# araffin/robotics-rl-srl

Measured on NVIDIA H100. Metric: env-steps/sec KukaButtonGymEnv-v0 ground_truth @4096 envs/GPU, higher is better.
Workload: dtype f32

## Files before the change

### robotics-rl-srl_b200/csrc/kuka_coop.cuh

```cuda
#pragma once
#include <math.h>
#include <stdint.h>
#include "kuka_params.cuh"

#if defined(__CUDACC__)
#define KC_F __device__ __forceinline__
#else
#define KC_F inline
#endif
#if defined(__CUDA_ARCH__)
#define KC_RSQRT(x) rsqrtf(x)
#else
#define KC_RSQRT(x) (1.0f / sqrtf(x))
#endif

#define KC_G 4
#define KC_BS 53
#define KC_CS 25

enum {
    KB_R = 0,
    KB_N = 0,
    KB_F = 3,
    KB_PM = 6,
// ... 344 lines not shown
    for (int t = 0; t < 4; ++t) {
        const int idx = 4 * u + t;
        const int f = idx < 10 ? KB_M + idx : KB_N + (idx - 10);
        float v[KK_NB];
#pragma unroll
        for (int j = 0; j < KK_NB; ++j) v[j] = s[j * KC_BS + f];
#pragma unroll
        for (int j = KK_NB - 1; j >= 1; --j) v[j == 10 ? 7 : j - 1] += v[j];
#pragma unroll
        for (int j = 0; j < KK_NB - 1; ++j)
            if (j != 9) s[j * KC_BS + f] = v[j];
    }
}
template <class S>
KC_F void kc_ph_mass(const S& s, int u) {
    kc3 a[KK_NB], pv[KK_NB];
#pragma unroll
    for (int i = 0; i < KK_NB; ++i) { a[i] = kc_ld3(s, i * KC_BS + KB_A); pv[i] = kc_ld3(s, i * KC_BS + KB_PV); }
#pragma unroll
    for (int k = 0; k < KK_NB / KC_G; ++k) {
        const int j = u + KC_G * k, o = j * KC_BS;
        const kc3 aj = kc_ld3(s, o + KB_A), pvj = kc_ld3(s, o + KB_PV);
        const kc3 h = kc_ld3(s, o + KB_H);
        s[KC_OFF_BIAS + j] = kc_dot(aj, kc_ld3(s, o + KB_N)) + kc_dot(pvj, kc_ld3(s, o + KB_F));
        float I[6];
#pragma unroll
        for (int t = 0; t < 6; ++t) I[t] = s[o + KB_IO + t];
        const kc3 Pm = kc_fma(s[o + KB_M], pvj, kc_cross(aj, h));
        const kc3 Lm = kc_add(kc_symv(I, aj), kc_cross(h, pvj));
#pragma unroll
        for (int i = 0; i < KK_NB; ++i) {
            if (i > 4 * k + 3) continue;
            const float val = kc_anc(i, j) ? kc_dot(a[i], Lm) + kc_dot(pv[i], Pm) : 0.f;
            if (i < 4 * k || i <= j) s[KC_OFF_MA + j * KC_MS + i] = val;
        }
    }
}

template <bool TWOB, bool SCALED, class S>
KC_F void kc_ph_rows(const S& s, const KukaParams& P, const float (&A)[KK_NB][KK_NB], int nc, int u, const float* tgt = nullptr) {
#pragma unroll 1
    for (int r = u; r < 3 * nc; r += KC_G) {
        const int c = r < nc ? r : (r - nc) >> 1;
        const int co = KC_OFF_CT + c * KC_CTS, ro = KC_OFF_ROWS + r * KC_RS;
        const kc3 n = kc_ld3(s, co + 3), pt = kc_ld3(s, co + 6);
        kc3 dir = n;
        if (r >= nc) {
            kc3 t1, t2;
            if (fabsf(n.z) > 0.70710678f) {
                const float a = n.y * n.y + n.z * n.z, kk = KC_RSQRT(a);
                t1 = kc_mk(0.f, -n.z * kk, n.y * kk); t2 = kc_mk(a * kk, -n.x * t1.z, n.x * t1.y);
            } else {
                const float a = n.x * n.x + n.y * n.y, kk = KC_RSQRT(a);
                t1 = kc_mk(-n.y * kk, n.x * kk, 0.f); t2 = kc_mk(-n.z * t1.y, n.z * t1.x, a * kk);
            }
            dir = ((r - nc) & 1) ? t2 : t1;
        }
        const int body = (int)s[co], shape = (int)s[co + 1];
        float J[KK_NB];
#pragma unroll
        for (int j = 0; j < KK_NB; ++j)
            J[j] = kc_anc(j, body) ? kc_dot(dir, kc_cross(kc_ld3(s, j * KC_BS + KB_A), kc_sub(pt, kc_ld3(s, j * KC_BS + KB_P)))) : 0.f;
        const float jb = shape == 1 ? -dir.z : 0.f, jb2 = TWOB && shape == 3 ? -dir.z : 0.f;
        float D = 0.f, off = 0.f;
#pragma unroll
        for (int i = 0; i < KK_NB; ++i) {
            float acc = 0.f;
#pragma unroll
            for (int j = 0; j < KK_NB; ++j) acc = fmaf(i >= j ? A[i][j] : A[j][i], J[j], acc);
            D = fmaf(J[i], acc, D);
            if (SCALED) off = fmaf(J[i], tgt[i], off);
            s[ro + KK_ROW_J + i] = SCALED ? J[i] * P.sat_isig[i] : J[i];
            s[ro + KK_ROW_W + i] = SCALED ? acc * P.sat_sig[i] : acc;
            if (SCALED && r < nc) s[KC_OFF_WT + 4 * i + r] = acc * P.sat_sig[i];
        }
        s[ro + KK_ROW_J + KK_NB] = jb; s[ro + KK_ROW_W + KK_NB] = jb * P.btn_minv;
        s[ro + KK_ROW_J + KK_NB + 1] = jb2; s[ro + KK_ROW_W + KK_NB + 1] = jb2 * P.btn_minv;
        D = fmaf(jb, jb * P.btn_minv, D);
        if (TWOB) D = fmaf(jb2, jb2 * P.btn_minv, D);
        s[ro + KK_ROW_INVD] = 1.0f / D;
        const float pen = s[co + 2];
        s[ro + KK_ROW_TGT] = (r < nc ? (pen > 0.f ? -pen * P.inv_dt : -P.erp * pen * P.inv_dt) : 0.f) - off;
    }
    if (SCALED && u >= nc) {
#pragma unroll
        for (int i = 0; i < KK_NB; ++i) s[KC_OFF_WT + 4 * i + u] = 0.f;
    }
}

#if defined(__CUDACC__)
#define KC_RUN(call) do { call; __syncwarp(gmask); } while (0)
#else
#define KC_RUN(call) do { for (int u = 0; u < KC_G; ++u) { call; } } while (0)
#endif

#if defined(__CUDACC__)
template <bool TWOB, class S>
KC_F bool kc_kinematics(const S& s, const float* tab, const KukaParams& P, const KcKinIn& in, int u, unsigned gmask) {
    KC_RUN(kc_ph_local(s, tab, in, u));
    KC_RUN(kc_ph_chain(s, tab, P, u));
    const bool near = kc_ph_body<TWOB>(s, tab, P, in, u);
    __syncwarp(gmask);
    if (near) KC_RUN((kc_ph_collect<TWOB>(s, tab, P, u)));
    return near;
}
#else
template <bool TWOB, class S>
KC_F bool kc_kinematics(const S& s, const float* tab, const KukaParams& P, const KcKinIn& in) {
    KC_RUN(kc_ph_local(s, tab, in, u));
    KC_RUN(kc_ph_chain(s, tab, P, u));
    bool near = false;
    for (int u = 0; u < KC_G; ++u) near = kc_ph_body<TWOB>(s, tab, P, in, u);
    if (near) KC_RUN((kc_ph_collect<TWOB>(s, tab, P, u)));
    return near;
}
#endif

#if defined(__CUDACC__)
template <class S>
KC_F void kc_dynamics(const S& s, const KukaParams& P, const float* qd, int u, unsigned gmask) {
#else
template <class S>
KC_F void kc_dynamics(const S& s, const KukaParams& P, const float* qd) {
#endif
    KC_RUN(kc_ph_vel_terms(s, qd, u));
    KC_RUN(kc_ph_prefix2(s, KB_W, KB_VO, 0.f, u));
    KC_RUN(kc_ph_acc_terms(s, qd, u));
    KC_RUN(kc_ph_prefix2(s, KB_AW, KB_AV, -P.gz, u));
    KC_RUN(kc_ph_wrench(s, P, u));
    KC_RUN(kc_ph_subtree(s, u));
    KC_RUN(kc_ph_mass(s, u));
}
```

### robotics-rl-srl_b200/csrc/kuka_device.cuh

```cuda
#pragma once
#include <math.h>
#include <stdint.h>
#include "kuka_params.cuh"
#include "philox.cuh"
#include "kuka_coop.cuh"

#define KK_DEV __device__ __forceinline__

#if defined(KK_TIMING)
#define KK_PROBE_D(d) kk_probe_any |= ((d) != 0.f);
#define KK_PROBE_SWEEP() { ++kk_probe_sweep; if (!kk_probe_any && !kk_probe_conv) kk_probe_conv = kk_probe_sweep; kk_probe_any = false; }
#else
#define KK_PROBE_D(d)
#define KK_PROBE_SWEEP()
#endif
enum { KK_PH_KIN = 0, KK_PH_IK, KK_PH_DYN, KK_PH_CHOL, KK_PH_SETUP, KK_PH_FAST, KK_PH_GENERAL, KK_PH_ENV, KK_NPH };
#if defined(KK_PHASES) && defined(__CUDACC__)
struct KkPhaseClock { long long last; long long acc[KK_NPH]; };
#define KK_PH(clk, k) do { if (clk) { const long long t_ = clock64(); (clk)->acc[k] += t_ - (clk)->last; (clk)->last = t_; } } while (0)
#else
struct KkPhaseClock { long long dummy; };
#define KK_PH(clk, k) do { (void)(clk); } while (0)
#endif
struct f3 { float x, y, z; };
struct alignas(16) kk_f4 { float x, y, z, w; };
KK_DEV f3 mk3(float x, float y, float z) { f3 r; r.x = x; r.y = y; r.z = z; return r; }
KK_DEV f3 operator+(f3 a, f3 b) { return mk3(a.x + b.x, a.y + b.y, a.z + b.z); }
KK_DEV f3 operator-(f3 a, f3 b) { return mk3(a.x - b.x, a.y - b.y, a.z - b.z); }
KK_DEV f3 operator*(float s, f3 a) { return mk3(s * a.x, s * a.y, s * a.z); }
KK_DEV float dot3(f3 a, f3 b) { return fmaf(a.x, b.x, fmaf(a.y, b.y, a.z * b.z)); }
KK_DEV f3 cross3(f3 a, f3 b) { return mk3(a.y * b.z - a.z * b.y, a.z * b.x - a.x * b.z, a.x * b.y - a.y * b.x); }
KK_DEV float norm3(f3 a) { return sqrtf(dot3(a, a)); }
KK_DEV f3 symv(const float* I, f3 v) {
    return mk3(I[0] * v.x + I[1] * v.y + I[2] * v.z, I[1] * v.x + I[3] * v.y + I[4] * v.z, I[2] * v.x + I[4] * v.y + I[5] * v.z);
}

#define KK_PAR(i) ((i) == 0 ? -1 : (i) == 10 ? 7 : (i) - 1)

struct KukaEnv {
    float q[KK_NB], qd[KK_NB];
    float qb, qdb;
    float ee[3];
    float bbx, bby, bbz;
    float bspeed;
    double by64;
    float tgt[3];
    float grip[3], eepos[3];
    int counter, n_contacts, n_outside, terminated;
    int cbutton, ctable;
    uint32_t episode, total_steps;
    float ep_ret; int ep_len;
    float qb2, qdb2;
    float bb2x, bb2y;
    int n_contacts2;
    int goal_id;
    int cany0, cany1;
};

struct KukaKin {
    f3 a[KK_NB];
    f3 p[KK_NB];
    f3 c[KK_NB];
    f3 pv[KK_NB];
    float Iw[KK_NB][6];
    float R6[9];
};

struct KukaContacts {
    int n;
    int body[KK_MAXC], shape[KK_MAXC];
    float dist[KK_MAXC];
    f3 nrm[KK_MAXC], pt[KK_MAXC];
};

KK_DEV void sphere_cylinder(f3 s, float r, float cx, float cy, float z0, float z1, float R, float& dist, f3& n) {
    const float dx = s.x - cx, dy = s.y - cy;
    const float rho = sqrtf(dx * dx + dy * dy);
    const f3 radial = rho > 1e-12f ? mk3(dx / rho, dy / rho, 0.f) : mk3(1.f, 0.f, 0.f);
    float d;
    if (s.z >= z1 || s.z <= z0) {
        const float zf = s.z >= z1 ? z1 : z0;
        if (rho <= R) { d = fabsf(s.z - zf); n = mk3(0.f, 0.f, s.z >= z1 ? 1.f : -1.f); }
        else { const f3 vec = mk3(dx - radial.x * R, dy - radial.y * R, s.z - zf); d = norm3(vec); n = (1.0f / d) * vec; }
    } else if (rho > R) {
        d = rho - R; n = radial;
    } else {
        const float d_top = z1 - s.z, d_side = R - rho;
        if (d_top <= d_side) { d = -d_top; n = mk3(0.f, 0.f, 1.f); } else { d = -d_side; n = radial; }
    }
    dist = d - r;
}

KK_DEV void kuka_world_frames(const KukaParams& P, const float* q, float (&Rb)[KK_NB][9], f3 (&pb)[KK_NB]) {
    float R[9] = {1.f, 0.f, 0.f, 0.f, 1.f, 0.f, 0.f, 0.f, 1.f}, R7[9]; f3 p = mk3(P.base[0], P.base[1], P.base[2]), p7 = p;
    for (int t = 0; t < 9; ++t) R7[t] = R[t];
    for (int b = 0; b < KK_NB; ++b) {
        if (b == 10) { for (int t = 0; t < 9; ++t) R[t] = R7[t]; p = p7; }
        const float ox = P.org[b][0], oy = P.org[b][1], oz = P.org[b][2];
        p = mk3(p.x + R[0] * ox + R[1] * oy + R[2] * oz, p.y + R[3] * ox + R[4] * oy + R[5] * oz, p.z + R[6] * ox + R[7] * oy + R[8] * oz);
        float sn, cs; sincosf(q[b], &sn, &cs);
        const float t = 1.f - cs, ax = P.axis[b][0], ay = P.axis[b][1], az = P.axis[b][2];
// ... 471 lines not shown
                    t1 = mk3(0.f, -n.z * kk, n.y * kk); t2 = mk3(a * kk, -n.x * t1.z, n.x * t1.y);
                } else {
                    const float a = n.x * n.x + n.y * n.y, kk = rsqrtf(a);
                    t1 = mk3(-n.y * kk, n.x * kk, 0.f); t2 = mk3(-n.z * t1.y, n.z * t1.x, a * kk);
                }
                dir = ((r - nc) & 1) ? t2 : t1;
            }
            const int body = ct.body[c];
            float J[KK_NB];
#pragma unroll
            for (int j = 0; j < KK_NB; ++j) {
                const bool anc = (j == body) || (j <= 7 && j < body) || (j == 8 && body == 9) || (j == 10 && body == 11);
                J[j] = anc ? dot3(dir, cross3(k.a[j], ct.pt[c] - k.p[j])) : 0.f;
            }
            float* row = cR[COOP ? 0 : r];
            float D = 0.f, off = 0.f;
#pragma unroll
            for (int i = 0; i < KK_NB; ++i) {
                float w = 0.f;
#pragma unroll
                for (int j = 0; j < KK_NB; ++j) w = fmaf(KK_A(i, j), J[j], w);
                D = fmaf(J[i], w, D); off = fmaf(J[i], tgt[i], off);
                row[KK_ROW_J + i] = J[i] * P.sat_isig[i];
                row[KK_ROW_W + i] = w * P.sat_sig[i];
            }
            const float jb = ct.shape[c] == 1 ? -dir.z : 0.f, jb2 = TWOB && ct.shape[c] == 3 ? -dir.z : 0.f;
            row[KK_ROW_J + KK_NB] = jb; row[KK_ROW_W + KK_NB] = jb * P.btn_minv;
            row[KK_ROW_J + KK_NB + 1] = jb2; row[KK_ROW_W + KK_NB + 1] = jb2 * P.btn_minv;
            D = fmaf(jb, jb * P.btn_minv, D);
            if (TWOB) D = fmaf(jb2, jb2 * P.btn_minv, D);
            row[KK_ROW_INVD] = 1.0f / D;
            c_lam[r] = 0.f;
            const float pen = ct.dist[c];
            row[KK_ROW_TGT] = (r < nc ? (pen > 0.f ? -pen * P.inv_dt : -P.erp * pen * P.inv_dt) : 0.f) - off;
        }
    }
#pragma unroll
    for (int i = 0; i < KK_NB; ++i)
#pragma unroll
        for (int j = 0; j <= i; ++j) A[i][j] *= P.sat_ss[i * (i + 1) / 2 + j];
#define KK_ROW_PTR(r) (COOP ? &sc[KC_OFF_ROWS + (r) * KC_RS] : cR[COOP ? 0 : (r)])
#define KK_ROW_LOAD4(dst, ptr, base)                                                                                   \
    _Pragma("unroll")                                                                                                  \
    for (int q4 = 0; q4 < 4; ++q4) {                                                                                   \
        const kk_f4 t4 = *reinterpret_cast<const kk_f4*>((ptr) + (base) + 4 * q4);                                   \
        dst[4 * q4] = t4.x; dst[4 * q4 + 1] = t4.y; dst[4 * q4 + 2] = t4.z; dst[4 * q4 + 3] = t4.w;                    \
    }
#define KK_ROW_DOT(Jr, out)                                                                                            \
    {                                                                                                                  \
        float p0 = Jr[0] * v[0], p1 = Jr[1] * v[1], p2 = Jr[2] * v[2], p3 = Jr[3] * v[3];                              \
        p0 = fmaf(Jr[4], v[4], p0); p1 = fmaf(Jr[5], v[5], p1); p2 = fmaf(Jr[6], v[6], p2); p3 = fmaf(Jr[7], v[7], p3); \
        p0 = fmaf(Jr[8], v[8], p0); p1 = fmaf(Jr[9], v[9], p1); p2 = fmaf(Jr[10], v[10], p2); p3 = fmaf(Jr[11], v[11], p3); \
        p0 = fmaf(Jr[12], v[12], p0);                                                                                  \
        if (TWOB) p1 = fmaf(Jr[13], v[ND - 1], p1);                                                                    \
        out = (p0 + p1) + (p2 + p3);                                                                                   \
    }
    const float bl_lo_hi = bl_lo ? P.lim_maximp : 0.f, bl_hi_hi = bl_hi ? P.lim_maximp : 0.f;
    const float b2l_lo_hi = b2l_lo ? P.lim_maximp : 0.f, b2l_hi_hi = b2l_hi ? P.lim_maximp : 0.f;
#define KK_BUTTON2_MOTOR()                                                                                             \
    if (TWOB) {                                                                                                        \
        const float s2 = fminf(fmaxf(fmaf(b2_tgt - v[ND - 1], b_invd, b2_lam), -b_hi), b_hi);                          \
        v[ND - 1] = fmaf(P.btn_minv, s2 - b2_lam, v[ND - 1]); b2_lam = s2;                                             \
    }
#define KK_BUTTON2_LIMITS()                                                                                            \
    if (TWOB) {                                                                                                        \
        float s2 = fminf(fmaxf(fmaf(b2l_lo_t - v[ND - 1], b_invd, b2l_lo_lam), 0.f), b2l_lo_hi);                       \
        v[ND - 1] = fmaf(P.btn_minv, s2 - b2l_lo_lam, v[ND - 1]); b2l_lo_lam = s2;                                     \
        s2 = fminf(fmaxf(fmaf(b2l_hi_t + v[ND - 1], b_invd, b2l_hi_lam), 0.f), b2l_hi_hi);                             \
        v[ND - 1] = fmaf(-P.btn_minv, s2 - b2l_hi_lam, v[ND - 1]); b2l_hi_lam = s2;                                    \
    }
#define KK_MOTOR_ROWS()                                                                                                \
    _Pragma("unroll")                                                                                                  \
    for (int i = 0; i < KK_NB; ++i) {                                                                                  \
        const float s = __saturatef(fmaf(-cs[i], v[i], lam[i]));                                                       \
        const float d = s - lam[i];                                                                                    \
        lam[i] += d;             \
        KK_PROBE_D(d)                                                                                                  \
        _Pragma("unroll")                                                                                              \
        for (int j = 0; j < KK_NB; ++j) v[j] = fmaf(KK_A(j, i), d, v[j]);                                              \
    }
#define KK_MOTOR_ROWS_WATCH()                                                                                          \
    _Pragma("unroll")                                                                                                  \
    for (int i = 0; i < KK_NB; ++i) {                                                                                  \
        const kk_f4 w4 = *reinterpret_cast<const kk_f4*>(wt + 4 * i);                                                  \
        const float s = __saturatef(fmaf(-cs[i], v[i], lam[i]));                                                       \
        const float d = s - lam[i];                                                                                    \
        lam[i] += d;                                                                                                   \
        KK_PROBE_D(d)                                                                                                  \
        _Pragma("unroll")                                                                                              \
        for (int j = 0; j < KK_NB; ++j) v[j] = fmaf(KK_A(j, i), d, v[j]);                                              \
        wjv[0] = fmaf(w4.x, d, wjv[0]); wjv[1] = fmaf(w4.y, d, wjv[1]); wjv[2] = fmaf(w4.z, d, wjv[2]); wjv[3] = fmaf(w4.w, d, wjv[3]); \
    }
    int it0 = 0;
#if defined(KK_TIMING)
    bool kk_probe_any = false; int kk_probe_sweep = 0, kk_probe_conv = 0;
#endif
    bool resume_mid_sweep = false;
    KK_PH(ph, KK_PH_SETUP);
    if ((lim_lo_mask | lim_hi_mask) == 0u) {
        float bminv, nbminv, lo_hi, hi_hi, lo_t, hi_t;
        asm volatile("mov.f32 %0, %1;" : "=f"(bminv) : "f"(P.btn_minv));
        asm volatile("mov.f32 %0, %1;" : "=f"(nbminv) : "f"(-P.btn_minv));
        asm volatile("mov.f32 %0, %1;" : "=f"(lo_hi) : "f"(bl_lo_hi));
        asm volatile("mov.f32 %0, %1;" : "=f"(hi_hi) : "f"(bl_hi_hi));
        asm volatile("mov.f32 %0, %1;" : "=f"(lo_t) : "f"(bl_lo_t));
        asm volatile("mov.f32 %0, %1;" : "=f"(hi_t) : "f"(bl_hi_t));
        bool act = false;
        bool more = true;
        int it = 0;
#define KK_SWEEP_BUTTONS()                                                                                               \
                {                 \
                    float s = fminf(fmaxf(fmaf(b_tgt - v[KK_NB], b_invd, b_lam), -b_hi), b_hi);                          \
                    v[KK_NB] = fmaf(bminv, s - b_lam, v[KK_NB]); b_lam = s;                                              \
                    s = fminf(fmaxf(fmaf(lo_t - v[KK_NB], b_invd, bl_lo_lam), 0.f), lo_hi);                              \
                    v[KK_NB] = fmaf(bminv, s - bl_lo_lam, v[KK_NB]); bl_lo_lam = s;                                      \
                    s = fminf(fmaxf(fmaf(hi_t + v[KK_NB], b_invd, bl_hi_lam), 0.f), hi_hi);                              \
                    v[KK_NB] = fmaf(nbminv, s - bl_hi_lam, v[KK_NB]); bl_hi_lam = s;                                     \
                }                                                                                                        \
                KK_BUTTON2_MOTOR() KK_BUTTON2_LIMITS()
        if (P.iters > 0) {
            int left = P.iters;
            asm volatile("mov.u32 %0, %0;" : "+r"(left));
#if defined(__CUDA_ARCH__)
            const bool quiet = __all_sync(__activemask(), nc == 0);
#else
            const bool quiet = false;
#endif
            if (quiet) {
#pragma unroll 1
                do { KK_SWEEP_BUTTONS() KK_MOTOR_ROWS() KK_PROBE_SWEEP() } while (--left > 0);
                it = P.iters;
            } else if constexpr (!COOP) {
#pragma unroll 1
                do {
                    KK_SWEEP_BUTTONS()
                    KK_MOTOR_ROWS()
                    KK_PROBE_SWEEP()
                    ++it;
                    more = --left > 0;
                    if (nc > 0) {
#pragma unroll 1
                        for (int c = 0; c < nc; ++c) {
                            const float* row = KK_ROW_PTR(c);
                            float Jr[16], jv;
                            KK_ROW_LOAD4(Jr, row, KK_ROW_J)
                            KK_ROW_DOT(Jr, jv)
                            act = act | (Jr[KK_ROW_TGT] - jv > 0.f);
                        }
                        if (act) more = false;
                    }
                } while (more);
            } else {
                const float* wt = &sc[KC_OFF_WT];
                float wjv[4], wthr[4], wjb[4], wjb2[4];
#pragma unroll
                for (int c = 0; c < 4; ++c) {
                    wjv[c] = 0.f; wthr[c] = -1e30f; wjb[c] = 0.f; wjb2[c] = 0.f;
                    if (c < nc) {
                        const float* row = KK_ROW_PTR(c);
                        float Jr[16];
                        KK_ROW_LOAD4(Jr, row, KK_ROW_J)
                        float p0 = Jr[0] * v[0], p1 = Jr[1] * v[1], p2 = Jr[2] * v[2], p3 = Jr[3] * v[3];
                        p0 = fmaf(Jr[4], v[4], p0); p1 = fmaf(Jr[5], v[5], p1); p2 = fmaf(Jr[6], v[6], p2); p3 = fmaf(Jr[7], v[7], p3);
                        p0 = fmaf(Jr[8], v[8], p0); p1 = fmaf(Jr[9], v[9], p1); p2 = fmaf(Jr[10], v[10], p2); p3 = fmaf(Jr[11], v[11], p3);
                        wjv[c] = (p0 + p1) + (p2 + p3);
                        wthr[c] = Jr[KK_ROW_TGT]; wjb[c] = Jr[KK_NB]; wjb2[c] = Jr[KK_NB + 1];
                    }
                }
                if (nc == 0) {
#pragma unroll
                    for (int i = 0; i < KK_NB; ++i) sc[KC_OFF_WT + 4 * i + u] = 0.f;
#if defined(__CUDACC__)
                    __syncwarp(gmask);
#endif
                }
#pragma unroll 1
                do {
                    KK_SWEEP_BUTTONS()
                    KK_MOTOR_ROWS_WATCH()
                    KK_PROBE_SWEEP()
                    ++it;
                    more = --left > 0;
#pragma unroll
                    for (int c = 0; c < 4; ++c) {
                        float jv = fmaf(wjb[c], v[KK_NB], wjv[c]);
                        if (TWOB) jv = fmaf(wjb2[c], v[ND - 1], jv);
                        act = act | (wthr[c] - jv > 0.f);
                    }
                    if (act) more = false;
                } while (more);
            }
        }
#undef KK_SWEEP_BUTTONS
        if (act) { it0 = it - 1; resume_mid_sweep = true; } else it0 = it;
#ifdef KK_TIMING
        if (dbg && nc > 0) *dbg |= 1u;
#endif
    }
    KK_PH(ph, KK_PH_FAST);
#ifdef KK_TIMING
    if (dbg) *dbg |= ((unsigned)kk_probe_conv & 255u) << 24;
    if (dbg) { *dbg |= ((unsigned)nc & 15u) << 2; if (lim_lo_mask | lim_hi_mask) *dbg |= 64u; if (it0 < P.iters) *dbg |= 2u | ((unsigned)(P.iters - it0) & 255u) << 8; }
#endif
    if (it0 < P.iters) {
#pragma unroll 1
        for (int it = it0; it < P.iters; ++it) {
            if (!resume_mid_sweep) {
            {
                const float s = fminf(fmaxf(fmaf(b_tgt - v[KK_NB], b_invd, b_lam), -b_hi), b_hi);
                v[KK_NB] = fmaf(P.btn_minv, s - b_lam, v[KK_NB]); b_lam = s;
            }
            KK_BUTTON2_MOTOR()
            KK_MOTOR_ROWS()
            {
                float s = fminf(fmaxf(fmaf(bl_lo_t - v[KK_NB], b_invd, bl_lo_lam), 0.f), bl_lo_hi);
                v[KK_NB] = fmaf(P.btn_minv, s - bl_lo_lam, v[KK_NB]); bl_lo_lam = s;
                s = fminf(fmaxf(fmaf(bl_hi_t + v[KK_NB], b_invd, bl_hi_lam), 0.f), bl_hi_hi);
                v[KK_NB] = fmaf(-P.btn_minv, s - bl_hi_lam, v[KK_NB]); bl_hi_lam = s;
            }
            KK_BUTTON2_LIMITS()
            }
            resume_mid_sweep = false;
            if (lim_lo_mask | lim_hi_mask) {
#pragma unroll
                for (int i = 0; i < KK_NB; ++i) {
                    if (lim_lo_mask & (1u << i)) {
                        const float t = -P.erp * (e.q[i] - P.lower[i]) * P.inv_dt;
                        const float s = fminf(fmaxf(fmaf(-invd[i] * P.sat_isig[i], v[i], fmaf(t - tgt[i], invd[i], lim_lam_lo[i])), 0.f), P.lim_maximp);
                        const float d = (s - lim_lam_lo[i]) * P.sat_isig[i]; lim_lam_lo[i] = s;
#pragma unroll
                        for (int j = 0; j < KK_NB; ++j) v[j] = fmaf(KK_A(j, i), d, v[j]);
                    }
                    if (lim_hi_mask & (1u << i)) {
                        const float t = -P.erp * (P.upper[i] - e.q[i]) * P.inv_dt;
                        const float s = fminf(fmaxf(fmaf(invd[i] * P.sat_isig[i], v[i], fmaf(t + tgt[i], invd[i], lim_lam_hi[i])), 0.f), P.lim_maximp);
                        const float d = (s - lim_lam_hi[i]) * P.sat_isig[i]; lim_lam_hi[i] = s;
#pragma unroll
                        for (int j = 0; j < KK_NB; ++j) v[j] = fmaf(-KK_A(j, i), d, v[j]);
                    }
                }
            }
#pragma unroll 1
            for (int r = 0; r < 3 * nc; ++r) {
                float lo = 0.f, hi = 1e10f;
                if (r >= nc) {
                    hi = P.mu * c_lam[(r - nc) >> 1]; lo = -hi;
                    if (hi == 0.f && c_lam[r] == 0.f) continue;
                }
                const float* row = KK_ROW_PTR(r);
                float Jr[16], Wr[16], jv;
                KK_ROW_LOAD4(Jr, row, KK_ROW_J)
                KK_ROW_LOAD4(Wr, row, KK_ROW_W)
                KK_ROW_DOT(Jr, jv)
                const float s = fminf(fmaxf(fmaf(Jr[KK_ROW_TGT] - jv, Jr[KK_ROW_INVD], c_lam[r]), lo), hi);
                const float d = s - c_lam[r];
                if (d == 0.f) continue;
                c_lam[r] = s;
#pragma unroll
                for (int j = 0; j < KK_NB + 1; ++j) v[j] = fmaf(Wr[j], d, v[j]);
                if (TWOB) v[ND - 1] = fmaf(Wr[KK_NB + 1], d, v[ND - 1]);
            }
        }
    }
    KK_PH(ph, KK_PH_GENERAL);
#undef KK_MOTOR_ROWS
#undef KK_MOTOR_ROWS_WATCH
#undef KK_ROW_PTR
#undef KK_ROW_LOAD4
#undef KK_ROW_DOT
#pragma unroll
    for (int i = 0; i < KK_NB; ++i) v[i] = fmaf(v[i], P.sat_isig[i], tgt[i]);
#pragma unroll
    for (int i = 0; i < KK_NB; ++i) { e.qd[i] = v[i]; e.q[i] = fmaf(P.dt, v[i], e.q[i]); }
    e.qdb = v[KK_NB]; e.qb = fmaf(P.dt, v[KK_NB], e.qb);
    if (TWOB) { e.qdb2 = v[ND - 1]; e.qb2 = fmaf(P.dt, v[ND - 1], e.qb2); }
    KK_PH(ph, KK_PH_SETUP);
}
```

### robotics-rl-srl_b200/csrc/kuka_kernels.cu

```cuda
#include <stdio.h>
#include <stdlib.h>
#include <string.h>
#include <vector>
#include "common.cuh"
#include "kuka_state.cuh"
#include "kuka_device.cuh"
#include "render_core.h"

struct KukaNext : KukaState {
    uint8_t* valid;
    int32_t* episode;
    uint8_t* progress;
    int helper;
};

namespace {

constexpr float DELTA_V = 0.03f, DELTA_V_CONTINUOUS = 0.0035f, DELTA_THETA = 0.1f;
constexpr double NOISE_STD = 0.01, NOISE_STD_CONTINUOUS = 0.0001, NOISE_STD_JOINTS = 0.002;
constexpr int N_CONTACTS_BEFORE_TERMINATION = 5, N_STEPS_OUTSIDE_SAFETY_SPHERE = 5000, N_RANDOM_ACTIONS_AT_INIT = 5;

template <bool CG, class T>
KK_DEV T ld_state(const T* p) { return CG ? __ldcg(p) : *p; }

// ... 48 lines not shown
KK_DEV void apply_ee_delta(const KukaParams& P, KukaEnv& e, float dx, float dy, float dz) {
    e.ee[0] = fminf(fmaxf(e.ee[0] + dx, P.box[0]), P.box[1]);
    e.ee[1] = fminf(fmaxf(e.ee[1] + dy, P.box[2]), P.box[3]);
    e.ee[2] = fminf(fmaxf(e.ee[2] + dz, P.box[4]), P.box[5]);
}

KK_DEV void reset_action(const KukaParams& P, const double* __restrict__ d17, uint64_t genv, uint32_t episode, int s,
                         float& dx, float& dy, float& dz) {
    dx = dy = dz = 0.f;
    if (d17) { dx = (float)d17[2 + 3 * s]; dy = (float)d17[3 + 3 * s]; dz = (float)d17[4 + 3 * s]; return; }
    const uint4 r = philox4x32_10(P.seed, genv, episode, PHILOX_PURPOSE_RESET0 + 1 + s);
    if (P.action_joints) {
        const double u1 = philox_u01(r.x, r.y), u2 = philox_u01(r.z, r.w);
        dx = (float)(0.1 * (7.0 + sqrt(-2.0 * log(1.0 - u1)) * cos(6.283185307179586 * u2)));
    } else if (P.is_discrete) {
        const float sign = philox_u01(r.x, r.y) > 0.5 ? 1.f : -1.f;
        const uint32_t idx = __umulhi(r.z, 3u);
        dx = idx == 0 ? sign * DELTA_V : 0.f; dy = idx == 1 ? sign * DELTA_V : 0.f; dz = idx == 2 ? sign * DELTA_V : 0.f;
    } else {
        const double u1 = philox_u01(r.x, r.y), u2 = philox_u01(r.z, r.w);
        const double z = sqrt(-2.0 * log(1.0 - u1)) * cos(6.283185307179586 * u2);
        const float sign = (3.0 + z) >= 0.0 ? 1.f : -1.f;
        dx = dy = dz = sign * DELTA_V_CONTINUOUS;
    }
}

template <bool TWOB>
KK_DEV void reset_begin(const KukaParams& P, KukaEnv& e, const double* __restrict__ d17, uint64_t genv) {
#pragma unroll
    for (int i = 0; i < KK_NB; ++i) { e.q[i] = P.snap_q[i]; e.qd[i] = P.snap_qd[i]; }
    e.ee[0] = P.snap_ee[0]; e.ee[1] = P.snap_ee[1]; e.ee[2] = P.snap_ee[2];
    e.qb = P.snap_qb; e.qdb = P.snap_qdb;
    e.bbx = P.btn_base[0]; e.bby = P.btn_base[1]; e.bbz = P.btn_base[2];
    e.bspeed = 0.f;
    if (P.moving_button) {
        if (d17) e.bspeed = (float)d17[17];
        else e.bspeed = (philox4x32_10(P.seed, genv, e.episode, PHILOX_PURPOSE_RESET0 + 6).x & 1u) ? 0.001f : -0.001f;
    }
    e.by64 = (double)P.btn_base[1];
    if (TWOB) {
        e.qb2 = P.snap_qb; e.qdb2 = P.snap_qdb;
        e.bb2x = P.btn_base[0]; e.bb2y = -P.btn_base[1];
        if (P.random_target) {
            if (d17) { e.bb2x = (float)d17[0]; e.bb2y = (float)d17[1]; }
            else {
                const uint4 r = philox4x32_10(P.seed, genv, e.episode, PHILOX_PURPOSE_RESET0);
                e.bb2x = (float)((double)P.btn_base[0] + (double)P.rand_x * (-1.0 + 2.0 * philox_u01(r.x, r.y)));
                e.bb2y = (float)(-(double)P.btn_base[1] + 0.175 * (-1.0 + philox_u01(r.z, r.w)));
            }
        }
        return;
    }
    if (P.random_target) {
        if (d17) { e.bbx = (float)d17[0]; e.bby = (float)d17[1]; e.by64 = d17[1]; }
        else {
            const uint4 r = philox4x32_10(P.seed, genv, e.episode, PHILOX_PURPOSE_RESET0);
            e.bbx = (float)((double)P.btn_base[0] + (double)P.rand_x * (-1.0 + 2.0 * philox_u01(r.x, r.y)));
            e.by64 = (double)P.btn_base[1] + (double)P.rand_y * (-1.0 + 2.0 * philox_u01(r.z, r.w));
            e.bby = (float)e.by64;
        }
    }
}

template <bool TWOB>
KK_DEV void reset_end(const KukaParams& P, KukaEnv& e) {
    e.tgt[0] = e.bbx; e.tgt[1] = e.bby;
    e.tgt[2] = e.bbz + P.glider_z + e.qb + P.target_h;
    if (TWOB) e.tgt[2] = P.two_tgt_z;
    if (TWOB) { e.n_contacts2 = 0; e.goal_id = 0; }
    e.counter = 0; e.n_contacts = 0; e.n_outside = 0; e.terminated = 0;
    e.ep_ret = 0.f; e.ep_len = 0;
    e.episode += 1;
}

enum { KUKA_OP_ROLLOUT = 0, KUKA_OP_RESET = 1, KUKA_OP_SETTLE = 2, KUKA_OP_PREFETCH = 3 };

#ifdef KK_TIMING
__device__ unsigned long long kk_timing[1 << 16];
#define KK_TIMING_RECORD() do { if (lead) kk_timing[(warp * (COOP ? 8 : 32) + slot) & 0xFFFF] = ((unsigned long long)(clock64() - kk_t0) << 32) | dbgf | (helper ? 1u << 18 : 0u); } while (0)
#else
#define KK_TIMING_RECORD() do { } while (0)
#endif
#ifdef KK_PHASES
__device__ unsigned long long kk_phase[1 << 13][KK_NPH + 1];
#endif
template <bool JOINTS, bool TWOB, bool PREFETCH = false, bool COOP = false, bool TRACE = false>
__global__ void __launch_bounds__(128, 1) kuka_kernel(const __grid_constant__ KukaDev d, int n, int op, int T,
                                                       const void* __restrict__ actions, const float* __restrict__ noise,
                                                       const uint8_t* __restrict__ mask, const double* __restrict__ draws,
                                                       float* __restrict__ obs, float* __restrict__ rew,
                                                       uint8_t* __restrict__ done, float* __restrict__ ep_ret,
                                                       int32_t* __restrict__ ep_len, float* __restrict__ snap, const KukaNext nx,
                                                       float4* __restrict__ trace, int* __restrict__ trace_len) {
    const int lane = threadIdx.x & 31, warp = (blockIdx.x * blockDim.x + threadIdx.x) >> 5;
#ifdef KK_TIMING
    const long long kk_t0 = clock64(); unsigned dbgf = 0u;
#endif
#ifdef KK_PHASES
    KkPhaseClock kk_ph_clk; KkPhaseClock* const ph = &kk_ph_clk; unsigned kk_nphys = 0u;
    kk_ph_clk.last = clock64();
#pragma unroll
    for (int k2 = 0; k2 < KK_NPH; ++k2) kk_ph_clk.acc[k2] = 0;
#else
    KkPhaseClock* const ph = nullptr;
#endif
    const int slot = COOP ? lane >> 2 : lane;
    const int u = COOP ? lane & 3 : 0;
    const bool lead = !COOP || u == 0;
    const unsigned gmask = COOP ? 0xFu << (lane & ~3) : 0u;
    extern __shared__ float4 kc_smem[];
    float* const kc_tab = reinterpret_cast<float*>(kc_smem);
    KcScratch sc;
    sc.b = reinterpret_cast<float*>(kc_smem) + ((KC_CONST_WORDS + 31) / 32) * 32 + (8 * (threadIdx.x >> 5) + (lane >> 2)) * KC_ES;
    if constexpr (COOP) {
        kc_fill_const(d.P, kc_tab, threadIdx.x, blockDim.x);
        __syncthreads();
    }
    int i = -1;
    if (slot < d.epw) { i = warp * d.epw + slot; if (i >= n) i = -1; }
    bool helper = false;
    if constexpr (PREFETCH) {
        if (nx.helper && op == KUKA_OP_ROLLOUT && slot == d.epw && slot < (COOP ? 8 : 32)) {
            int pick = -1;
            if (lead) {
                int best = -1;
                for (int k2 = 0; k2 < d.epw; ++k2) {
                    const int j = warp * d.epw + k2;
                    if (j < n && !reinterpret_cast<volatile const uint8_t*>(nx.valid)[j]) {
                        const int pr = nx.progress[j];
                        if (pr > best) { best = pr; pick = j; }
                    }
                }
            }
            if (COOP) pick = __shfl_sync(gmask, pick, lane & ~3);
            if (pick >= 0) { i = pick; helper = true; op = KUKA_OP_PREFETCH; }
        }
    }
    if (i < 0) return;
    if (op == KUKA_OP_RESET && mask && !mask[i]) return;
    if constexpr (PREFETCH) { if (op == KUKA_OP_PREFETCH && !helper && nx.valid[i]) return; }
    const KukaParams& P = d.P;
    const uint64_t genv = P.env_offset + (uint64_t)i;
    const size_t N = (size_t)n;
    KukaEnv e; KukaKin k; KukaContacts ct;
    env_load<TWOB>(d, i, e);
    int nc_reg = 0;
    if constexpr (PREFETCH) {
        __syncwarp();
    }

    int reset_left = 0;
    bool in_reset = false;
    bool pending = false;
    int rep = 0, t = 0;
    int saved_cb = 0, saved_ct = 0, saved_a0 = 0, saved_a1 = 0;
    float dx = 0.f, dy = 0.f, dz = 0.f;
    float qj[JOINTS ? 7 : 1];
#pragma unroll
    for (int j = 0; j < (JOINTS ? 7 : 1); ++j) qj[j] = 0.f;
    const double* d17 = nullptr;
    if (op == KUKA_OP_RESET) {
        d17 = draws ? draws + (size_t)i * (TRACE ? KUKA_DIST_DRAWS : 18) : nullptr;
        reset_begin<TWOB>(P, e, d17, genv);
        in_reset = true; reset_left = N_RANDOM_ACTIONS_AT_INIT;
    } else if (op == KUKA_OP_SETTLE) {
#pragma unroll
        for (int j = 0; j < KK_NB; ++j) { e.q[j] = P.snap_q[j]; e.qd[j] = 0.f; }
        e.ee[0] = P.ee_init[0]; e.ee[1] = P.ee_init[1]; e.ee[2] = P.ee_init[2];
        e.qb = 0.f; e.qdb = 0.f; e.bbx = P.btn_base[0]; e.bby = P.btn_base[1]; e.bbz = P.btn_base[2]; e.bspeed = 0.f; e.by64 = 0.0;
        if (TWOB) { e.qb2 = 0.f; e.qdb2 = 0.f; e.bb2x = P.btn_base[0]; e.bb2y = -P.btn_base[1]; }
        in_reset = true; reset_left = 500;
    }
    int ms = 0;
    bool consumed = false;
    bool partial = false;
    int budget = T;
    if constexpr (PREFETCH) {
        if (op == KUKA_OP_PREFETCH) {
            const int prog = helper ? (int)nx.progress[i] : 0;
            if (prog > 0 && nx.episode[i] == (int)e.episode) {
                env_load<TWOB, true>(nx, i, e);
                in_reset = true; reset_left = N_RANDOM_ACTIONS_AT_INIT - prog;
            } else {
                if (helper && lead) nx.episode[i] = (int)e.episode;
                reset_begin<TWOB>(P, e, nullptr, genv);
                in_reset = true; reset_left = N_RANDOM_ACTIONS_AT_INIT;
            }
        }
    }
    auto leave = [&]() {
        e.cbutton = saved_cb; e.ctable = saved_ct;
        if (TWOB) { e.cany0 = saved_a0; e.cany1 = saved_a1; }
        KK_TIMING_RECORD();
        if constexpr (TRACE) { if (lead && op != KUKA_OP_SETTLE) trace_len[i] = ms; }
#ifdef KK_PHASES
        KK_PH(ph, KK_PH_ENV);
        if (lead) {
            unsigned long long* const kp = kk_phase[(warp * (COOP ? 8 : 32) + slot) & ((1 << 13) - 1)];
#pragma unroll
            for (int k2 = 0; k2 < KK_NPH; ++k2) kp[k2] = (unsigned long long)kk_ph_clk.acc[k2];
            kp[KK_NPH] = kk_nphys;
        }
#endif
        if constexpr (PREFETCH) {
            if (op == KUKA_OP_PREFETCH) {
                if (!lead) return;
                env_store<TWOB>(nx, i, e);
                if (partial) { nx.progress[i] = (uint8_t)(N_RANDOM_ACTIONS_AT_INIT - reset_left); return; }
                nx.episode[i] = (int)e.episode - 1;
                nx.progress[i] = 0;
                __threadfence();
                reinterpret_cast<volatile uint8_t*>(nx.valid)[i] = 1;
                return;
            }
        }
        if (lead) env_store<TWOB>(d, i, e);
    };
    bool fin = false, settled = false;
#define KK_LEAVE_LOOP() { if (COOP) { leave(); fin = true; continue; } else break; }
    for (;;) {
        if constexpr (COOP) {
            if (__all_sync(0xffffffffu, fin)) break;
            if (fin) continue;
        }
        if constexpr (COOP) {
            KcKinIn kin;
#pragma unroll
            for (int j = 0; j < KK_NB; ++j) kin.q[j] = e.q[j];
            kin.qb = e.qb; kin.qb2 = e.qb2; kin.bbx = e.bbx; kin.bby = e.bby; kin.bbz = e.bbz; kin.bb2x = e.bb2x; kin.bb2y = e.bb2y;
            KK_PH(ph, KK_PH_ENV);
            __syncwarp(gmask);
            const bool near = kc_kinematics<TWOB>(sc, kc_tab, P, kin, u, gmask);
            e.grip[0] = sc[8 * KC_BS + KB_C]; e.grip[1] = sc[8 * KC_BS + KB_C + 1]; e.grip[2] = sc[8 * KC_BS + KB_C + 2];
            e.eepos[0] = sc[6 * KC_BS + KB_P]; e.eepos[1] = sc[6 * KC_BS + KB_P + 1]; e.eepos[2] = sc[6 * KC_BS + KB_P + 2];
            const int fl = near ? (int)sc[KC_OFF_LINK + 6] : 0;
            e.cbutton = fl & 1; e.ctable = (fl >> 1) & 1;
            if (TWOB) { e.cany0 = (fl >> 2) & 1; e.cany1 = (fl >> 3) & 1; }
            nc_reg = near ? (int)sc[KC_OFF_LINK + 7] : 0;
            KK_PH(ph, KK_PH_KIN);
        } else { KK_PH(ph, KK_PH_ENV); kuka_fk<TWOB>(P, e, k, ct); KK_PH(ph, KK_PH_KIN); }
        const int new_cb = e.cbutton, new_ct = e.ctable, new_a0 = TWOB ? e.cany0 : 0, new_a1 = TWOB ? e.cany1 : 0;
        if (pending) {
            pending = false;
            const size_t off = (size_t)t * N + (size_t)i;
            const float ddx = e.tgt[0] - e.grip[0], ddy = e.tgt[1] - e.grip[1], ddz = e.tgt[2] - e.grip[2];
            const float distance = sqrtf(ddx * ddx + ddy * ddy + ddz * ddz);
            float reward;
            if (TWOB) {
                const int contact = e.goal_id ? saved_a1 : saved_a0;
                reward = 0.f;
                if (e.goal_id) { e.n_contacts2 += contact; reward = contact ? 1.f : 0.f; }
                else {
                    e.n_contacts += contact;
                    if (e.n_contacts >= N_CONTACTS_BEFORE_TERMINATION) { e.goal_id = 1; e.tgt[0] = e.bb2x; e.tgt[1] = e.bb2y; }
                }
                if (distance > P.max_distance || saved_ct) { reward = -1.f; e.n_outside += 1; } else e.n_outside = 0;
                if (saved_ct || e.n_contacts2 >= N_CONTACTS_BEFORE_TERMINATION || e.n_outside >= N_STEPS_OUTSIDE_SAFETY_SPHERE - 1) e.terminated = 1;
                if (P.shape_reward) {
                    const int n_goal = e.goal_id ? e.n_contacts2 : e.n_contacts;
                    if (e.terminated && reward > 0.f) reward = 50.f;
                    else if (n_goal < N_CONTACTS_BEFORE_TERMINATION && contact) reward = 25.f;
                    else if (saved_ct) reward = -250.f;
                    else if (distance > P.max_distance) reward = -20.f;
                    else reward = -distance;
                }
            } else {
            reward = saved_cb ? 1.f : 0.f;
            e.n_contacts += saved_cb;
            if (distance > P.max_distance || saved_ct) { reward = -1.f; e.n_outside += 1; } else e.n_outside = 0;
            if (saved_ct || e.n_contacts >= N_CONTACTS_BEFORE_TERMINATION || e.n_outside >= N_STEPS_OUTSIDE_SAFETY_SPHERE) e.terminated = 1;
            if (P.shape_reward) {
                if (P.is_discrete) reward = -distance;
                else if (e.terminated && reward > 0.f) reward = 50.f;
                else if (e.terminated && reward < 0.f) reward = -250.f;
                else reward = -distance;
            }
            }
            const bool is_done = e.terminated || e.counter > P.max_steps;
#ifdef KK_TIMING
            if (is_done) dbgf |= 1u << 16;
#endif
            e.ep_ret += reward; e.ep_len += 1;
            if (rew && lead) rew[off] = reward;
            if (done && lead) done[off] = is_done ? 1 : 0;
// ... 570 lines not shown
```

Before: 107.8 million.

## Split watched contact rows across cooperative lanes with ballot-based activation check

In the fast PGS path's watch mode, each of the four cooperating lanes now tracks only its own contact row (one wjv accumulator, twelve per-lane weights held in registers) instead of every lane tracking all four rows through shared-memory float4 loads. Activation is decided with a warp ballot masked to the group. This removes the per-iteration shared loads and three quarters of the watch arithmetic, and drops the zeroing of unused weight slots. The cost is a ballot per sweep, more registers for the weights, and added phase-profiling counters that only exist in profiling builds.

```diff
diff --git a/robotics-rl-srl_b200/csrc/kuka_coop.cuh b/robotics-rl-srl_b200/csrc/kuka_coop.cuh
--- a/robotics-rl-srl_b200/csrc/kuka_coop.cuh
+++ b/robotics-rl-srl_b200/csrc/kuka_coop.cuh
@@ -450,10 +450,6 @@
         const float pen = s[co + 2];
         s[ro + KK_ROW_TGT] = (r < nc ? (pen > 0.f ? -pen * P.inv_dt : -P.erp * pen * P.inv_dt) : 0.f) - off;
     }
-    if (SCALED && u >= nc) {
-#pragma unroll
-        for (int i = 0; i < KK_NB; ++i) s[KC_OFF_WT + 4 * i + u] = 0.f;
-    }
 }
 
 #if defined(__CUDACC__)
diff --git a/robotics-rl-srl_b200/csrc/kuka_device.cuh b/robotics-rl-srl_b200/csrc/kuka_device.cuh
--- a/robotics-rl-srl_b200/csrc/kuka_device.cuh
+++ b/robotics-rl-srl_b200/csrc/kuka_device.cuh
@@ -14,9 +14,9 @@
 #define KK_PROBE_D(d)
 #define KK_PROBE_SWEEP()
 #endif
-enum { KK_PH_KIN = 0, KK_PH_IK, KK_PH_DYN, KK_PH_CHOL, KK_PH_SETUP, KK_PH_FAST, KK_PH_GENERAL, KK_PH_ENV, KK_NPH };
+enum { KK_PH_KIN = 0, KK_PH_IK, KK_PH_DYN, KK_PH_CHOL, KK_PH_SETUP, KK_PH_FAST_QUIET, KK_PH_FAST_WATCH, KK_PH_GENERAL, KK_PH_ENV, KK_NPH };
 #if defined(KK_PHASES) && defined(__CUDACC__)
-struct KkPhaseClock { long long last; long long acc[KK_NPH]; };
+struct KkPhaseClock { long long last; long long acc[KK_NPH]; unsigned nwatch; };
 #define KK_PH(clk, k) do { if (clk) { const long long t_ = clock64(); (clk)->acc[k] += t_ - (clk)->last; (clk)->last = t_; } } while (0)
 #else
 struct KkPhaseClock { long long dummy; };
@@ -654,20 +654,20 @@
 #define KK_MOTOR_ROWS_WATCH()                                                                                          \
     _Pragma("unroll")                                                                                                  \
     for (int i = 0; i < KK_NB; ++i) {                                                                                  \
-        const kk_f4 w4 = *reinterpret_cast<const kk_f4*>(wt + 4 * i);                                                  \
         const float s = __saturatef(fmaf(-cs[i], v[i], lam[i]));                                                       \
         const float d = s - lam[i];                                                                                    \
         lam[i] += d;                                                                                                   \
         KK_PROBE_D(d)                                                                                                  \
         _Pragma("unroll")                                                                                              \
         for (int j = 0; j < KK_NB; ++j) v[j] = fmaf(KK_A(j, i), d, v[j]);                                              \
-        wjv[0] = fmaf(w4.x, d, wjv[0]); wjv[1] = fmaf(w4.y, d, wjv[1]); wjv[2] = fmaf(w4.z, d, wjv[2]); wjv[3] = fmaf(w4.w, d, wjv[3]); \
+        wjv = fmaf(wl[i], d, wjv);                                                                                     \
     }
     int it0 = 0;
 #if defined(KK_TIMING)
     bool kk_probe_any = false; int kk_probe_sweep = 0, kk_probe_conv = 0;
 #endif
     bool resume_mid_sweep = false;
+    bool watching = false;
     KK_PH(ph, KK_PH_SETUP);
     if ((lim_lo_mask | lim_hi_mask) == 0u) {
         float bminv, nbminv, lo_hi, hi_hi, lo_t, hi_t;
@@ -677,6 +677,9 @@
         asm volatile("mov.f32 %0, %1;" : "=f"(hi_hi) : "f"(bl_hi_hi));
         asm volatile("mov.f32 %0, %1;" : "=f"(lo_t) : "f"(bl_lo_t));
         asm volatile("mov.f32 %0, %1;" : "=f"(hi_t) : "f"(bl_hi_t));
+        asm volatile("mov.f32 %0, %0;" : "+f"(b_hi));
+#pragma unroll
+        for (int i = 0; i < KK_NB; ++i) asm volatile("mov.f32 %0, %0;" : "+f"(cs[i]));
         bool act = false;
         bool more = true;
         int it = 0;
@@ -698,6 +701,7 @@
 #else
             const bool quiet = false;
 #endif
+            watching = !quiet;
             if (quiet) {
 #pragma unroll 1
                 do { KK_SWEEP_BUTTONS() KK_MOTOR_ROWS() KK_PROBE_SWEEP() } while (--left > 0);
@@ -723,28 +727,20 @@
                     }
                 } while (more);
             } else {
-                const float* wt = &sc[KC_OFF_WT];
-                float wjv[4], wthr[4], wjb[4], wjb2[4];
-#pragma unroll
-                for (int c = 0; c < 4; ++c) {
-                    wjv[c] = 0.f; wthr[c] = -1e30f; wjb[c] = 0.f; wjb2[c] = 0.f;
-                    if (c < nc) {
-                        const float* row = KK_ROW_PTR(c);
-                        float Jr[16];
-                        KK_ROW_LOAD4(Jr, row, KK_ROW_J)
-                        float p0 = Jr[0] * v[0], p1 = Jr[1] * v[1], p2 = Jr[2] * v[2], p3 = Jr[3] * v[3];
-                        p0 = fmaf(Jr[4], v[4], p0); p1 = fmaf(Jr[5], v[5], p1); p2 = fmaf(Jr[6], v[6], p2); p3 = fmaf(Jr[7], v[7], p3);
-                        p0 = fmaf(Jr[8], v[8], p0); p1 = fmaf(Jr[9], v[9], p1); p2 = fmaf(Jr[10], v[10], p2); p3 = fmaf(Jr[11], v[11], p3);
-                        wjv[c] = (p0 + p1) + (p2 + p3);
-                        wthr[c] = Jr[KK_ROW_TGT]; wjb[c] = Jr[KK_NB]; wjb2[c] = Jr[KK_NB + 1];
-                    }
-                }
-                if (nc == 0) {
-#pragma unroll
-                    for (int i = 0; i < KK_NB; ++i) sc[KC_OFF_WT + 4 * i + u] = 0.f;
-#if defined(__CUDACC__)
-                    __syncwarp(gmask);
-#endif
+                float wl[KK_NB], wjv = 0.f, wthr = -1e30f, wjb = 0.f, wjb2 = 0.f;
+#pragma unroll
+                for (int i = 0; i < KK_NB; ++i) wl[i] = 0.f;
+                if (u < nc) {
+                    const float* row = KK_ROW_PTR(u);
+                    float Jr[16];
+                    KK_ROW_LOAD4(Jr, row, KK_ROW_J)
+                    float p0 = Jr[0] * v[0], p1 = Jr[1] * v[1], p2 = Jr[2] * v[2], p3 = Jr[3] * v[3];
+                    p0 = fmaf(Jr[4], v[4], p0); p1 = fmaf(Jr[5], v[5], p1); p2 = fmaf(Jr[6], v[6], p2); p3 = fmaf(Jr[7], v[7], p3);
+                    p0 = fmaf(Jr[8], v[8], p0); p1 = fmaf(Jr[9], v[9], p1); p2 = fmaf(Jr[10], v[10], p2); p3 = fmaf(Jr[11], v[11], p3);
+                    wjv = (p0 + p1) + (p2 + p3);
+                    wthr = Jr[KK_ROW_TGT]; wjb = Jr[KK_NB]; wjb2 = Jr[KK_NB + 1];
+#pragma unroll
+                    for (int i = 0; i < KK_NB; ++i) wl[i] = sc[KC_OFF_WT + 4 * i + u];
                 }
 #pragma unroll 1
                 do {
@@ -753,12 +749,13 @@
                     KK_PROBE_SWEEP()
                     ++it;
                     more = --left > 0;
-#pragma unroll
-                    for (int c = 0; c < 4; ++c) {
-                        float jv = fmaf(wjb[c], v[KK_NB], wjv[c]);
-                        if (TWOB) jv = fmaf(wjb2[c], v[ND - 1], jv);
-                        act = act | (wthr[c] - jv > 0.f);
-                    }
+                    float jv = fmaf(wjb, v[KK_NB], wjv);
+                    if (TWOB) jv = fmaf(wjb2, v[ND - 1], jv);
+#if defined(__CUDA_ARCH__)
+                    act = (__ballot_sync(__activemask(), wthr - jv > 0.f) & gmask) != 0u;
+#else
+                    act = wthr - jv > 0.f;
+#endif
                     if (act) more = false;
                 } while (more);
             }
@@ -769,7 +766,10 @@
         if (dbg && nc > 0) *dbg |= 1u;
 #endif
     }
-    KK_PH(ph, KK_PH_FAST);
+#if defined(KK_PHASES) && defined(__CUDACC__)
+    if (ph && watching) ++ph->nwatch;
+#endif
+    KK_PH(ph, watching ? KK_PH_FAST_WATCH : KK_PH_FAST_QUIET);
 #ifdef KK_TIMING
     if (dbg) *dbg |= ((unsigned)kk_probe_conv & 255u) << 24;
     if (dbg) { *dbg |= ((unsigned)nc & 15u) << 2; if (lim_lo_mask | lim_hi_mask) *dbg |= 64u; if (it0 < P.iters) *dbg |= 2u | ((unsigned)(P.iters - it0) & 255u) << 8; }
diff --git a/robotics-rl-srl_b200/csrc/kuka_kernels.cu b/robotics-rl-srl_b200/csrc/kuka_kernels.cu
--- a/robotics-rl-srl_b200/csrc/kuka_kernels.cu
+++ b/robotics-rl-srl_b200/csrc/kuka_kernels.cu
@@ -154,7 +154,7 @@
 #define KK_TIMING_RECORD() do { } while (0)
 #endif
 #ifdef KK_PHASES
-__device__ unsigned long long kk_phase[1 << 13][KK_NPH + 1];
+__device__ unsigned long long kk_phase[1 << 13][KK_NPH + 2];
 #endif
 template <bool JOINTS, bool TWOB, bool PREFETCH = false, bool COOP = false, bool TRACE = false>
 __global__ void __launch_bounds__(128, 1) kuka_kernel(const __grid_constant__ KukaDev d, int n, int op, int T,
@@ -173,6 +173,7 @@
     kk_ph_clk.last = clock64();
 #pragma unroll
     for (int k2 = 0; k2 < KK_NPH; ++k2) kk_ph_clk.acc[k2] = 0;
+    kk_ph_clk.nwatch = 0u;
 #else
     KkPhaseClock* const ph = nullptr;
 #endif
@@ -272,6 +273,7 @@
 #pragma unroll
             for (int k2 = 0; k2 < KK_NPH; ++k2) kp[k2] = (unsigned long long)kk_ph_clk.acc[k2];
             kp[KK_NPH] = kk_nphys;
+            kp[KK_NPH + 1] = kk_ph_clk.nwatch;
         }
 #endif
         if constexpr (PREFETCH) {
```

Result: faster. 112.6 million (median of 6 runs) (+4.4%).
